# jimmyshe/liorf

Hardware: AMD Instinct MI355X
Metric: LM iterations/sec (64-line scan vs 200k-pt map) (higher is better)
Workload: dtype f32; 1 GPU; kitti64: 120000-pt scan vs 200000-pt local surf map, 30 LM iterations per scan (early exit off), one scan per GPU at a time, 8 distinct seeded scans in rotation, map replicated; n_q=120000, n_m=200000, distinct_scans=8, parallelism=scan-per-gpu x1

## Files before the change

liorf_amd/csrc/s2m_abi.hip:

```cpp
#include <hip/hip_runtime.h>

#include <cfloat>
#include <cmath>
#include <cstdio>
#include <cstdlib>
#include <cstring>
#include <algorithm>
#include <limits>
#include <map>
#include <new>
#include <string>
#include <vector>

#include "s2m_context.hpp"
#include "s2m_kernels.hpp"

using namespace s2m;
using namespace s2m::host;

namespace {

inline uint32_t host_f2ord(float f) { uint32_t u; memcpy(&u, &f, 4); return (u & 0x80000000u) ? ~u : (u | 0x80000000u); }
inline float host_ord2f(uint32_t o) { uint32_t u = (o & 0x80000000u) ? (o & 0x7fffffffu) : ~o; float f; memcpy(&f, &u, 4); return f; }

// ... 305 lines not shown
    SlotTable tbl;
    int nslots = 1;
    int nblocks = 0;
    int table_cap = 0;
    int wpb = kBlock / 64;
    bool batch = false;
    bool split = false;
    bool late = false;
    bool split_auto = false;
};

LoopShape shape_of(s2m_context* h)
{
    LoopShape sh;
    memset(&sh.tbl, 0, sizeof(sh.tbl));
    sh.tbl.ctx[0] = h->reg.dctx.as<DevCtx>();
    sh.tbl.st[0] = h->reg.state.as<DevState>();
    sh.nslots = 1; sh.nblocks = h->hctx.nblocks; sh.table_cap = h->hctx.table_cap; sh.wpb = h->hctx.wpb;
    sh.batch = h->batch.parent != nullptr && !h->batch.slot_mode;
    sh.split = h->tune.split_mode == 1;
    return sh;
}

template <bool HOOK, int NW, int MINW, int MODE, int CNW>
inline void launch_k(hipStream_t s, const LoopShape& sh, int L, int flags, int grid_x = 0)
{
    hipLaunchKernelGGL((k_register<HOOK, NW, MINW, MODE, CNW>), dim3(grid_x > 0 ? std::min(grid_x, sh.nblocks) : sh.nblocks, sh.nslots), dim3(NW * 64), 0, s,
                       sh.tbl, L, flags);
}

inline void launch_fused(s2m_context* h, const LoopShape& sh, bool hook, int L, int solve_prev)
{
// ... 510 lines not shown
    key.push_back(part); key.push_back(part ? h->tune.seg_iters : 0);
    for (int b : live) { key.push_back(b); key.push_back(h->batch.kids[(size_t)b]->hctx.table_cap); key.push_back(h->batch.kids[(size_t)b]->hctx.wpb); }
    auto it = h->batch.graphs.find(key);
    if (it != h->batch.graphs.end()) { *out = it->second; return S2M_OK; }
    hipGraph_t graph = nullptr;
    hipGraphExec_t exec = nullptr;
    std::vector<LoopShape> loops;
    if (h->tune.lockstep) {
        for (int wpb : { kBlock / 64, kBigWaves }) {
            LoopShape sh;
            memset(&sh.tbl, 0, sizeof(sh.tbl));
            sh.nslots = 0; sh.wpb = wpb; sh.batch = true;
            for (int b : live) {
                s2m_context* k = h->batch.kids[(size_t)b];
                if (k->hctx.wpb != wpb) continue;
                sh.tbl.ctx[sh.nslots] = k->reg.dctx.as<DevCtx>();
                sh.tbl.st[sh.nslots] = k->reg.state.as<DevState>();
                sh.nslots++;
                sh.nblocks = std::max(sh.nblocks, k->hctx.nblocks);
                sh.table_cap = std::max(sh.table_cap, k->hctx.table_cap);
            }
            sh.split = h->tune.split_mode == 1;
            sh.split_auto = h->tune.split_mode == 2 || h->tune.split_mode < 0;
            if (sh.nslots) loops.push_back(sh);
        }
    } else
        for (int b : live) loops.push_back(shape_of(h->batch.kids[(size_t)b]));
    S2M_HIP(h, hipStreamBeginCapture(h->stream, hipStreamCaptureModeThreadLocal));
    bool ok = hipEventRecord(h->batch.ev_fork, h->stream) == hipSuccess;
    hipStream_t keep = h->stream;
    for (size_t j = 0; j < loops.size(); j++) {
        hipStream_t br = h->batch.branch_streams[j];
// ... 658 lines not shown
```

liorf_amd/csrc/s2m_kernels.hpp:

```cpp
#pragma once
#include <float.h>
#include <math.h>
#include <string.h>
#include "s2m_types.h"

#if defined(__HIPCC__)
#define S2M_HD __host__ __device__
#else
#define S2M_HD
#endif

namespace s2m {

template <typename T> using gptr = __attribute__((address_space(1))) T*;
template <typename T> __device__ __forceinline__ gptr<T> G(T* p) { return (gptr<T>)p; }
typedef float v4f __attribute__((ext_vector_type(4)));
typedef const __attribute__((address_space(4))) DevCtx* CtxP;
__device__ __forceinline__ CtxP ctx_const(const DevCtx* p) { return (CtxP)p; }
__device__ __forceinline__ GridDesc grid_of(CtxP cp)
{
    GridDesc g;
    g.ox = cp->g.ox; g.oy = cp->g.oy; g.oz = cp->g.oz; g.inv_e = cp->g.inv_e; g.e = cp->g.e;
    g.nx = cp->g.nx; g.ny = cp->g.ny; g.nz = cp->g.nz; g.ncells = cp->g.ncells;
    return g;
}
__device__ __forceinline__ uint32_t f2ord(float f)
{
    uint32_t u = __float_as_uint(f);
    return (u & 0x80000000u) ? ~u : (u | 0x80000000u);
}

__device__ __forceinline__ int cell_coord(float v, float o, float inv_e, int n)
{
    float f = floorf((v - o) * inv_e);
    f = fminf(fmaxf(f, 0.0f), (float)(n - 1));
    return (int)f;
}

__device__ __forceinline__ void swap_if(bool c, float& a, float& b)
{
    float t = a; a = c ? b : a; b = c ? t : b;
}
__device__ __forceinline__ void swap_if(bool c, int& a, int& b)
{
    int t = a; a = c ? b : a; b = c ? t : b;
}

struct SincosfTable { double sign[4]; double hpi_inv, hpi, c0, c1, c2, c3, c4, s1, s2, s3; };
S2M_HD inline const SincosfTable& sincosf_table(int negate)
{
    static constexpr SincosfTable T[2] = {
        { { 1.0, -1.0, -1.0, 1.0 }, 0x1.45F306DC9C883p+23, 0x1.921FB54442D18p0, 0x1p0, -0x1.ffffffd0c621cp-2, 0x1.55553e1068f19p-5,
          -0x1.6c087e89a359dp-10, 0x1.99343027bf8c3p-16, -0x1.555545995a603p-3, 0x1.1107605230bc4p-7, -0x1.994eb3774cf24p-13 },
        { { 1.0, -1.0, -1.0, 1.0 }, 0x1.45F306DC9C883p+23, 0x1.921FB54442D18p0, -0x1p0, 0x1.ffffffd0c621cp-2, -0x1.55553e1068f19p-5,
          0x1.6c087e89a359dp-10, -0x1.99343027bf8c3p-16, -0x1.555545995a603p-3, 0x1.1107605230bc4p-7, -0x1.994eb3774cf24p-13 } };
    return T[negate];
}
S2M_HD inline uint32_t abstop12(float x)
{
    uint32_t u;
    memcpy(&u, &x, 4);
    return (u >> 20) & 0x7ffu;
}
S2M_HD inline float sinf_poly(double x, double x2, const SincosfTable& p, int n)
{
    if ((n & 1) == 0) {
        const double x3 = x * x2, s1 = p.s2 + x2 * p.s3, x7 = x3 * x2, s = x + x3 * p.s1;
        return (float)(s + x7 * s1);
    }
    const double x4 = x2 * x2, c2 = p.c3 + x2 * p.c4, c1 = p.c0 + x2 * p.c1, x6 = x4 * x2, c = c1 + x4 * p.c2;
    return (float)(c + x6 * c2);
}
S2M_HD inline float glibc_sincosf(float y, int which)
{
    double x = (double)y;
    if (abstop12(y) < abstop12(0x1.921FB6p-1f)) {
        if (abstop12(y) < abstop12(0x1p-12f)) return which ? 1.0f : y;
        return sinf_poly(x, x * x, sincosf_table(0), which);
    }
    if (abstop12(y) < abstop12(120.0f)) {
        const SincosfTable& p0 = sincosf_table(0);
        const double r = x * p0.hpi_inv;
        const int n = ((int32_t)r + 0x800000) >> 24;
        x = x - (double)n * p0.hpi;
        const double sgn = p0.sign[n & 3];
        return sinf_poly(x * sgn, x * x, sincosf_table((n & 2) ? 1 : 0), n ^ which);
    }
    return which ? (float)cos(x) : (float)sin(x);
}

S2M_HD inline void glibc_sincosf_both(float y, float& sn, float& cs)
{
    double x = (double)y;
    int n = 0;
    int tbl = 0;
    if (abstop12(y) < abstop12(0x1.921FB6p-1f)) {
        if (abstop12(y) < abstop12(0x1p-12f)) { sn = y; cs = 1.0f; return; }
    } else if (abstop12(y) < abstop12(120.0f)) {
        const SincosfTable& p0 = sincosf_table(0);
        const double r = x * p0.hpi_inv;
        n = ((int32_t)r + 0x800000) >> 24;
        x = x - (double)n * p0.hpi;
        x = x * p0.sign[n & 3];
        tbl = (n & 2) ? 1 : 0;
    } else { sn = (float)sin(x); cs = (float)cos(x); return; }
    const SincosfTable& p = sincosf_table(tbl);
    const double x2 = x * x;
    const float a = sinf_poly(x, x2, p, 0), b = sinf_poly(x, x2, p, 1);
    sn = (n & 1) ? b : a;
    cs = (n & 1) ? a : b;
}

S2M_HD inline float glibc_atanf(float x)
{
    const float atanhi[4] = { 4.6364760399e-01f, 7.8539812565e-01f, 9.8279368877e-01f, 1.5707962513e+00f };
    const float atanlo[4] = { 5.0121582440e-09f, 3.7748947079e-08f, 3.4473217170e-08f, 7.5497894159e-08f };
    const float aT[11] = { 3.3333334327e-01f, -2.0000000298e-01f, 1.4285714924e-01f, -1.1111110449e-01f, 9.0908870101e-02f, -7.6918758452e-02f,
                           6.6610731184e-02f, -5.8335702866e-02f, 4.9768779427e-02f, -3.6531571299e-02f, 1.6285819933e-02f };
    uint32_t u;
    memcpy(&u, &x, 4);
    const int32_t hx = (int32_t)u, ix = hx & 0x7fffffff;
    int id;
    if (ix >= 0x4c000000) {
        if (ix > 0x7f800000) return x + x;
        return (hx > 0) ? atanhi[3] + atanlo[3] : -atanhi[3] - atanlo[3];
// ... 494 lines not shown
        *n_waves_out = nw;
        if (st) st->n_waves = nw;
    }
    if (factor) for (int c = threadIdx.x; c < n_chunks; c += 1024) factor[c] = 0;
}

__global__ __launch_bounds__(1024) void k_chunk_table(const PrepTable tbl)
{
    const PrepSlot& ps = tbl.s[blockIdx.y];
    if (ps.n <= 0) return;
    chunk_table_body(ps.chunk_parts, ps.n, ps.n_chunks, ps.capacity, ps.wave_table, ps.n_waves, nullptr, nullptr);
}

__global__ __launch_bounds__(1024) void k_chunk_table_density(const SlotTable tbl)
{
    DevCtx* __restrict__ cp = const_cast<DevCtx*>(tbl.ctx[blockIdx.y]);
    DevState* __restrict__ st = tbl.st[blockIdx.y];
    if (!cp->density_pending) return;
    __syncthreads();
    if (threadIdx.x == 0) cp->density_pending = 0;
    chunk_table_body(cp->chunk_parts, cp->n_q, cp->n_chunks, cp->table_cap, cp->wave_table_rw, cp->n_waves_rw,
                     cp->chunk_factor, st);
}

__device__ __forceinline__ void plane_fit_5x3(float (&qr)[5][3], float (&x)[3])
{
    float hC[3], nU[3], nD[3];
    int perm[3] = { 0, 1, 2 };
#pragma unroll
    for (int k = 0; k < 3; k++) {
        float s = 0.0f;
#pragma unroll
// ... 396 lines not shown
            L[i][j] = v / dj;
        }
    }
    return true;
}

struct LmShared {
    double part[kFinThreads / 32][32];
    double tot[32];
    float  AtA[36], AtB[6];
    float  eA[6][6], eV[6][6], eVi[6][6], eV2[6][6], eW[6];
    int    eR[6], eC[6];
};

struct NoHook { __device__ __forceinline__ void operator()() const {} };
template <int NT, bool kFull, typename Early = NoHook, typename Late = NoHook>
__device__ __forceinline__ bool lm_close_iteration(CtxP cp, gptr<DevState> st, int nb_act, int iter,
                                                   bool writer, bool ne_only, const float (&pose0)[6], int degen0,
                                                   LmShared& sh, float* s_out, float (&pose_out)[6],
                                                   unsigned long long* stamps = nullptr,
                                                   Early early = Early(), Late late = Late())
{
    constexpr int NG = NT / 32;
    const auto trace = G(cp->trace);
    const int t = threadIdx.x, col = t & 31, grp = t >> 5, lane = t & 63, wave = t >> 6;
    double s = 0.0;
    if (col < kAcc) {
        const int nbk = cp->nblocks;
        const auto P = G((const double*)cp->partials) + (size_t)(iter & 1) * (size_t)nbk * kAcc;
        const int nb = min(nbk, nb_act);
        for (int b0 = grp; b0 < nb; b0 += 16 * NG) {
            double v[16];
#pragma unroll
            for (int u = 0; u < 16; u++) { const int b = b0 + u * NG; v[u] = (b < nb) ? P[(size_t)b * kAcc + col] : 0.0; }
#pragma unroll
            for (int u = 0; u < 16; u++) s += v[u];
        }
    }
    sh.part[grp][col] = s;
    __syncthreads();
    if (stamps) stamps[0] = wall_clock64();
    early();

    int n_sel = 0;
    if (wave == 0) {
        if (t < kAcc) {
// ... 120 lines not shown
    const float ang = (lane == 0) ? pose[2] : ((lane == 1) ? pose[1] : pose[0]);
    float snf, csf;
    glibc_sincosf_both(ang, snf, csf);
    const float B = __int_as_float(__builtin_amdgcn_readlane(__float_as_int(snf), 0)), A = __int_as_float(__builtin_amdgcn_readlane(__float_as_int(csf), 0));
    const float D = __int_as_float(__builtin_amdgcn_readlane(__float_as_int(snf), 1)), C = __int_as_float(__builtin_amdgcn_readlane(__float_as_int(csf), 1));
    const float F = __int_as_float(__builtin_amdgcn_readlane(__float_as_int(snf), 2)), E = __int_as_float(__builtin_amdgcn_readlane(__float_as_int(csf), 2));
    const float DE = D * E, DF = D * F;
    T[0] = A * C; T[1] = A * DF - B * E; T[2]  = B * F + A * DE; T[3]  = pose[3];
    T[4] = B * C; T[5] = A * E + B * DF; T[6]  = B * DE - A * F; T[7]  = pose[4];
    T[8] = -D;    T[9] = C * F;          T[10] = C * E;          T[11] = pose[5];
    sc6[0] = B; sc6[1] = A; sc6[2] = D; sc6[3] = C; sc6[4] = F; sc6[5] = E;
}

__global__ __launch_bounds__(256) void k_wave_density(const SlotTable tbl, int raw_limit)
{
    const CtxP cp = ctx_const(tbl.ctx[blockIdx.y]);
    const auto st = G((const DevState*)tbl.st[blockIdx.y]);
    const int lane = threadIdx.x & 63;
    const int wv = blockIdx.x * 4 + (threadIdx.x >> 6);
    if (!cp->density_pending || wv >= st->n_waves) return;
    const auto tb = G((const int2*)cp->wave_table);
    const int2 e = make_int2(tb[wv].x, tb[wv].y);
    const int i = e.x + lane;
    const bool valid = lane < e.y && i < cp->n_q;
    float sx = 0.0f, sy = 0.0f, sz = 0.0f;
    if (valid) {
        const float px = G(cp->qx)[i], py = G(cp->qy)[i], pz = G(cp->qz)[i];
        sx = ((st->T[0] * px + st->T[1] * py) + st->T[2]  * pz) + st->T[3];
        sy = ((st->T[4] * px + st->T[5] * py) + st->T[6]  * pz) + st->T[7];
        sz = ((st->T[8] * px + st->T[9] * py) + st->T[10] * pz) + st->T[11];
    }
    const bool fin = valid && (fabsf(sx) < 3.0e38f) && (fabsf(sy) < 3.0e38f) && (fabsf(sz) < 3.0e38f);
// ... 12 lines not shown
    for (int r = lane; r < nyb * nzb; r += 64) {
        const int zq = r / nyb;
        const int gcell = ((bz0 + zq) * g.ny + by0 + (r - zq * nyb)) * g.nx;
        raw += cell_start[gcell + bx1 + 1] - cell_start[gcell + bx0];
    }
    raw = __builtin_amdgcn_readlane(wave_incl_scan_i32(raw), 63);
    int f = raw <= raw_limit ? 1 : (raw <= 2 * raw_limit ? 2 : (raw <= 4 * raw_limit ? 4 : 8));
    f = min(f, max(e.y / 8, 1));
    if (lane == 0 && f > 1) atomicMax(&cp->chunk_factor[e.x >> 6], f);
}

#include "s2m_register.hpp"

__global__ __launch_bounds__(kFinThreads) void k_finalize(const SlotTable tbl, int iter, int mode)
{
    const CtxP cp = ctx_const(tbl.ctx[blockIdx.y]);
    const auto st = G(tbl.st[blockIdx.y]);
    const int done0 = st->done, degen0 = st->isDegenerate;
    const int nb_act = (st->n_waves + cp->wpb - 1) / cp->wpb;
    float pose0[6];
#pragma unroll
    for (int k = 0; k < 6; k++) pose0[k] = st->pose2[iter & 1][k];
    if (mode == 0 && done0) return;
    __shared__ LmShared sh;
    __shared__ float s_out[8];
    if (mode == 0 && threadIdx.x == 0 && cp->wl_count) { cp->wl_count[0] = 0; cp->wl_count[1] = 0; }
    float pose[6];
    const bool ended = lm_close_iteration<kFinThreads, true>(cp, st, nb_act, iter, true, mode == 1, pose0, degen0, sh, s_out, pose);
    if (mode == 0 && !ended && threadIdx.x < 64) {
        float T[12], sc6[6];
        build_transform(pose, (int)threadIdx.x, T, sc6);
        if (threadIdx.x == 0 && !st->stalled) {
#pragma unroll
            for (int k = 0; k < 12; k++) st->T[k] = T[k];
#pragma unroll
            for (int k = 0; k < 6; k++) st->sc[k] = sc6[k];
            st->T_valid = 1;
        }
    }
}

__global__ __launch_bounds__(256) void k_debug_sincos(const float* __restrict__ x, int n, float* __restrict__ s, float* __restrict__ c,
                                                      float* __restrict__ a)
// ... 298 lines not shown
```

liorf_amd/csrc/s2m_register.hpp:

```cpp
#pragma once

constexpr float kCertMargin = 2e-6f;
constexpr float kNbrReach   = 0.15f;
constexpr float kTightBound = 0.62f;
constexpr float kNbrReachCold = 0.10f;
constexpr int   kWalkLanes = 64;
constexpr int   kNbr = kNbrCap;
constexpr float kFragileSlack = 3e-5f;
constexpr float kSlabRound = 1e-6f;
constexpr float kAbsRound = 2.4e-7f;
constexpr int   kTilePad = 32;
constexpr int   kShareMin = 24;
constexpr int   kWalkMax = 384;
constexpr int   kServeLanes = 4;
typedef int v4i __attribute__((ext_vector_type(4)));
typedef float v3f __attribute__((ext_vector_type(3)));

__device__ __forceinline__ uint32_t key_hi(uint64_t k) { return (uint32_t)(k >> 32); }
__device__ __forceinline__ uint32_t key_lo(uint64_t k) { return (uint32_t)k; }
__device__ __forceinline__ void cas_u64(uint64_t& a, uint64_t& b)
{
    const bool c = b < a;
    const uint64_t t = a;
    a = c ? b : a; b = c ? t : b;
// ... 975 lines not shown
{
    sx = ((T[0] * px + T[1] * py) + T[2]  * pz) + T[3];
    sy = ((T[4] * px + T[5] * py) + T[6]  * pz) + T[7];
    sz = ((T[8] * px + T[9] * py) + T[10] * pz) + T[11];
    const bool fin = valid && (fabsf(sx) < 3.0e38f) && (fabsf(sy) < 3.0e38f) && (fabsf(sz) < 3.0e38f);
    const float ex = sx - cert.x, ey = sy - cert.y, ez = sz - cert.z;
    eps = sqrtf((ex * ex + ey * ey) + ez * ez) * 1.0001f + 1e-6f;
    return fin && !(!(ablate & 1) && (eps < cert.w));
}

template <int NW, int EPW, int MINW>
__global__ __launch_bounds__(NW / EPW * 64, MINW) void k_certify_lean(const SlotTable tbl, int launch)
{
    static_assert(NW % EPW == 0, "whole entries per wave");
    constexpr int NWL = NW / EPW;
    const CtxP cp = ctx_const(tbl.ctx[blockIdx.y]);
    const auto st = G(tbl.st[blockIdx.y]);
    const int done = st->done, n_waves = st->n_waves;
    if (done) return;
    __shared__ double red[NW][32];
    __shared__ float park[EPW == 2 ? NWL : 1][7][64];
    const int tid = threadIdx.x, lane = tid & 63, wave = tid >> 6;
    const int nblocks = cp->nblocks;
    const int nb_act = min((n_waves + NW - 1) / NW, nblocks);
    const int b = (int)blockIdx.x;
    if (b >= nb_act) return;
    const int nq = cp->n_q;
    const int ablate = cp->ablate;
    const bool single = nb_act * NW >= n_waves;
    static_assert(EPW == 1 || EPW == 2, "one or two entries per wave");
    const auto tb = G((const int2*)cp->wave_table);
    int2 chunkA = make_int2(0, 0), chunkB = make_int2(0, 0);
    {
// ... 5 lines not shown
    }
    float px = 0.0f, py = 0.0f, pz = 0.0f, bx = 0.0f, by = 0.0f, bz = 0.0f;
    v4f cert = { 0, 0, 0, 0 }, certB = { 0, 0, 0, 0 }, plane0 = { NAN, 0, 0, 0 };
    if (lane < chunkA.y && chunkA.x + lane < nq) {
        const int i = chunkA.x + lane;
        px = G(cp->qx)[i]; py = G(cp->qy)[i]; pz = G(cp->qz)[i];
        cert = G((const v4f*)cp->cert)[i];
        plane0 = G((const v4f*)cp->plane_cache)[i];
    }
    if (EPW == 2 && lane < chunkB.y && chunkB.x + lane < nq) {
        const int i = chunkB.x + lane;
        bx = G(cp->qx)[i]; by = G(cp->qy)[i]; bz = G(cp->qz)[i];
        certB = G((const v4f*)cp->cert)[i];
    }
    float T[12], sc6[6];
    if (st->T_valid) {
#pragma unroll
        for (int k = 0; k < 12; k++) T[k] = st->T[k];
#pragma unroll
        for (int k = 0; k < 6; k++) sc6[k] = st->sc[k];
    } else {
        float pose[6];
#pragma unroll
        for (int k = 0; k < 6; k++) pose[k] = st->pose2[launch & 1][k];
        build_transform(pose, lane, T, sc6);
    }
#pragma unroll
    for (int k = 0; k < 12; k++) T[k] = __int_as_float(__builtin_amdgcn_readfirstlane(__float_as_int(T[k])));
#pragma unroll
    for (int k = 0; k < 6; k++) sc6[k] = __int_as_float(__builtin_amdgcn_readfirstlane(__float_as_int(sc6[k])));

    bool defer = !single;
    int2 chunk = chunkA;
#pragma unroll 1
    for (int q = 0; q < EPW && single; q++) {
        const int w = wave + q * NWL;
        const int e = w * nb_act + b;
#pragma unroll
        for (int k = 0; k < 6; k++) asm volatile("" : "+s"(sc6[k]));
// ... 92 lines not shown
        if (tid == 0) {
            const int slot = atomicAdd(cp->wl_count + (launch & 1), 1);
            G(cp->wl_items)[(size_t)(launch & 1) * (size_t)nblocks + slot] = b;
        }
        return;
    }
    write_partial_row<NW>(cp, launch, b, tid, red);
}

template <bool HOOK, int NW, int MINW, int MODE, int CNW = NW>
__global__ __launch_bounds__(NW * 64, MINW) void k_register(const SlotTable tbl, int launch, int flags)
{
    static_assert(MODE == kSearch || CNW == NW, "only the search kernel works on another kernel's partition");
    static_assert(CNW % NW == 0, "a search workgroup takes the waves of a row in whole rounds");
    static_assert(!(HOOK && MODE == kCertify), "the observation hook needs the association in line");
    const CtxP cp = ctx_const(tbl.ctx[blockIdx.y]);
    const auto st = G(tbl.st[blockIdx.y]);
    const int done = st->done, n_waves = st->n_waves;
    if (!HOOK && done) return;
    const bool solve_prev = MODE != kSearch && (flags & kFlagSolvePrev) != 0;
    unsigned long long tk_start = 0, clk1 = 0, clk2 = 0;
    unsigned long long lm_stamps[7] = { 0, 0, 0, 0, 0, 0, 0 };
    if (HOOK) tk_start = wall_clock64();

    constexpr bool kHasSearch = MODE != kCertify;
    constexpr int  kTileWaves = kHasSearch ? NW : 1;
    __shared__ v4f     s_pts[kTileWaves][kHasSearch ? kTilePts : 1];
    static_assert(sizeof(v4f) * kTilePts >= sizeof(int32_t) * 18 * 64, "run table must fit the tile area");
    __shared__ double  red[CNW][32];
    __shared__ int2    s_rows[kTileWaves][kHasSearch ? 64 : 1];
    constexpr bool kKeep = kHasSearch && NW == 8 && MINW == 2;
    __shared__ float   s_keep[kKeep ? NW : 1][kKeep ? 7 : 1][kKeep ? 64 : 1];
    __shared__ float   s_lm_out[8];
    __shared__ LmShared s_lm;

    const int tid = threadIdx.x, lane = tid & 63, wave = tid >> 6;
    const int nblocks = cp->nblocks;
    const int nb_act = min((n_waves + CNW - 1) / CNW, nblocks);
    int b = (int)blockIdx.x;
    int wl_cnt = 0, wl_at = (int)blockIdx.x;
    const bool listed = MODE == kSearch && !(flags & kFlagAll);
    if (listed) {
        const auto wlc = G(cp->wl_count);
        wl_cnt = wlc[launch & 1];
        if (b == 0 && tid == 0) { wlc[(launch + 1) & 1] = 0; st->deferred_total += wl_cnt; }
    } else if (MODE == kSearch) {
        if (b == 0 && tid == 0) G(cp->wl_count)[(launch + 1) & 1] = 0;
    }
    for (;;) {
    if (listed) {
        if (wl_at >= wl_cnt) {
            if (!(flags & kFlagCloseAfter)) return;
// ... 18 lines not shown
    chunk.y = __builtin_amdgcn_readfirstlane(chunk.y);
    float px = 0.0f, py = 0.0f, pz = 0.0f;
    v4f cert = { 0, 0, 0, 0 }, plane0 = { NAN, 0, 0, 0 };
    const bool valid0 = lane < chunk.y && chunk.x + lane < nq;
    if (valid0) {
        const int i = chunk.x + lane;
        px = G(cp->qx)[i]; py = G(cp->qy)[i]; pz = G(cp->qz)[i];
        cert = G((const v4f*)cp->cert)[i];
        plane0 = G((const v4f*)cp->plane_cache)[i];
    }

    Fragile frag;
#pragma unroll
    for (int k = 0; k < 6; k++) frag.fr[k] = v4f{ 0.0f, 0.0f, 0.0f, 0.0f };
    float T[12], sc6[6];
    if (!solve_prev && st->T_valid) {
#pragma unroll
        for (int k = 0; k < 12; k++) T[k] = st->T[k];
#pragma unroll
        for (int k = 0; k < 6; k++) sc6[k] = st->sc[k];
    } else {
        float pose[6];
        if (solve_prev) {
            static_assert(MODE == kCertify || sizeof(LmShared) <= sizeof(v4f) * kTilePts * NW, "LM scratch must fit the tile area");
            LmShared& sh = (MODE == kCertify) ? s_lm : *reinterpret_cast<LmShared*>(&s_pts[0][0]);
            const int degen0 = st->isDegenerate;
            float pose0[6];
#pragma unroll
            for (int k = 0; k < 6; k++) pose0[k] = st->pose2[(launch - 1) & 1][k];
            if (HOOK) lm_stamps[5] = wall_clock64();
            auto early = [&]() {
                if (!HOOK && valid0 && !(cert.w > kFragileSlack) && !(ablate & 3)) {
                    const int i = chunk.x + lane;
                    frag.on = true;
                    frag.aux = G((const v4i*)cp->aux)[i];
#pragma unroll
                    for (int j = 0; j < 5; j++) frag.opos[j] = G(cp->npos)[(size_t)j * nq + i];
#pragma unroll
                    for (int j = 0; j < 6; j++) frag.fr[j] = G((const v4f*)cp->front)[(size_t)j * nq + i];
#pragma unroll
                    for (int j = 0; j < 5; j++) frag.alt[j] = G(cp->npos_alt)[(size_t)j * nq + i];
                    frag.alt_plane = G((const v4f*)cp->plane_alt)[i];
                }
            };
            auto late = [&]() {};
            const bool ended = lm_close_iteration<NW * 64, false>(cp, st, nb_act, launch - 1, blockIdx.x == 0, false, pose0, degen0,
                                                                 sh, s_lm_out, pose, HOOK ? lm_stamps : nullptr, early, late);
            if (ended) return;
        } else {
#pragma unroll
            for (int k = 0; k < 6; k++) pose[k] = st->pose2[launch & 1][k];
        }
        build_transform(pose, lane, T, sc6);
    }
#pragma unroll
    for (int k = 0; k < 12; k++) T[k] = __int_as_float(__builtin_amdgcn_readfirstlane(__float_as_int(T[k])));
#pragma unroll
    for (int k = 0; k < 6; k++) sc6[k] = __int_as_float(__builtin_amdgcn_readfirstlane(__float_as_int(sc6[k])));
    if (HOOK) lm_stamps[6] = wall_clock64();

    WaveProf prof;
    double acc[kAcc];
    bool defer = false;

    if (MODE == kSearch && CNW != NW) {
        for (int r = 0; r < CNW / NW; r++) {
// ... 194 lines not shown
        __syncthreads();
    write_partial_row<CNW>(cp, launch, b, tid, red);
    if (!listed) return;
    wl_at += (int)gridDim.x;
    __syncthreads();
    }
    if (MODE == kSearch) {
        __syncthreads();
        LmShared& sh = *reinterpret_cast<LmShared*>(&s_pts[0][0]);
        static_assert(MODE != kSearch || sizeof(LmShared) <= sizeof(v4f) * kTilePts * NW, "LM scratch must fit the tile area");
        float pose0[6], pose[6];
#pragma unroll
        for (int k = 0; k < 6; k++) pose0[k] = st->pose2[launch & 1][k];
        const int degen0 = st->isDegenerate;
        if (tid == 0) { cp->wl_count[0] = 0; cp->wl_count[1] = 0; }
        const bool ended = lm_close_iteration<NW * 64, false>(cp, st, nb_act, launch, true, false, pose0, degen0, sh, s_lm_out, pose);
        if (!ended && tid < 64) {
            float Tn[12], scn[6];
            build_transform(pose, tid, Tn, scn);
            if (tid == 0 && !st->stalled) {
#pragma unroll
                for (int k = 0; k < 12; k++) st->T[k] = Tn[k];
#pragma unroll
                for (int k = 0; k < 6; k++) st->sc[k] = scn[k];
                st->T_valid = 1;
            }
        }
    }
}
```

liorf_amd/csrc/s2m_types.h:

```cpp
#pragma once
#include <stdint.h>
#include <hip/hip_runtime.h>
#include "../../include/liorf_s2m.h"
#include "../../include/liorf_s2m_debug.h"

namespace s2m {

constexpr int kBlock = 512;
constexpr int kAcc = 28;
constexpr int kFinThreads = 1024;
constexpr int kMaxIter = 64;
constexpr int kProfWords = 32;
constexpr int kBlocksQuantum = 8;
constexpr int kNbrCap = 6;
constexpr int kMaxBlocks = 512;
constexpr int kBigWaves = 16;

struct GridDesc {
    float ox, oy, oz;
    float inv_e;
    float e;
    int   nx, ny, nz;
    int   ncells;
};

struct DevState {
    float pose[6];
    float pose2[2][6];
    float T[12];
    float sc[6];
    float matP[36];
    float AtA[36];
    float AtB[6];
    int32_t isDegenerate;
    int32_t done;
    int32_t converged;
    int32_t iters_run;
    int32_t n_sel_last;
    int32_t stalled;
    int32_t n_waves;
    int32_t T_valid;
    int32_t deferred_total;
    int32_t pad_;
};

struct DevCtx {
    GridDesc g;
    const float4* map_sorted;
    const int32_t* cell_start;
    const float* qx; const float* qy; const float* qz;
    const int32_t* qperm;
    int32_t* npos;
    float4*  cert;
    int4*    aux;
    float4*  front;
    float4*  plane_cache;
    float4*  plane_alt;
    int32_t* npos_alt;
    int32_t n_q, n_m, nblocks;
    int32_t wpb;
    int32_t table_cap;
    const int2* wave_table;
    const int32_t* n_waves;
    int2*    wave_table_rw; int32_t* n_waves_rw;
    const int32_t* chunk_parts;
    int32_t* chunk_factor;
    int32_t  n_chunks;
    int32_t  density_pending;
    double* partials;
    int32_t* wl_count;
    int32_t* wl_items;
    DevState* state;
    s2m_iter_trace* trace;
    float  gate_f;
    float  gate_r;
    double gate_sq, plane_tol, weight_scale, weight_min, conv_deg, conv_cm;
    float  eig_thresh;
    int32_t min_corr, max_iter, early_exit;
    int32_t tune[4];
    int32_t ablate;
    int32_t* dbg_idx5; float* dbg_d2; uint8_t* dbg_flag; float* dbg_coeff;
    unsigned long long* dbg_clk;
};

constexpr int kMaxSlots = 64;
struct SlotTable {
    const DevCtx* ctx[kMaxSlots];
    DevState*     st[kMaxSlots];
};

struct PrepSlot {
    const unsigned char* pts; size_t stride;
    int32_t n, n_chunks, base_parts, capacity, npb;
    int32_t *cell_of, *rank_of, *block_hist, *counts, *cell_start;
    float *qx, *qy, *qz; int32_t* qperm; float4* cert; int4* aux;
    int32_t* chunk_parts; int2* wave_table; int32_t* n_waves;
};
constexpr int kPrepSlots = 16;
struct PrepTable { PrepSlot s[kPrepSlots]; };

struct StateInit {
    DevState* dst; const int32_t* n_waves;
    float pose[6], T[12], sc[6], matP[36];
    int32_t isDegenerate;
// ... 8 lines not shown
```

liorf_amd/s2m.py:

```python
from __future__ import annotations

import ctypes as C
import importlib.util
import os
import sys

import numpy as np

_HERE = os.path.dirname(os.path.abspath(__file__))
LIB_PATH = os.environ.get("S2M_LIB") or os.path.join(_HERE, "libliorf_s2m.so")

S2M_OK = 0
S2M_ERR_CAPACITY = -5
ERRORS = {-1: "S2M_ERR_INVALID_ARG", -2: "S2M_ERR_NO_DEVICE", -3: "S2M_ERR_HIP", -4: "S2M_ERR_NO_SCAN",
          -5: "S2M_ERR_CAPACITY"}

ABI_SYMBOLS = [
    "s2m_version", "s2m_default_params", "s2m_create", "s2m_destroy", "s2m_last_error", "s2m_set_params", "s2m_get_params",
    "s2m_set_map", "s2m_set_map_device", "s2m_set_scan", "s2m_set_scan_device",
    "s2m_optimize", "s2m_optimize_resident", "s2m_optimize_launch", "s2m_optimize_collect",
    "s2m_optimize_batch", "s2m_batch_set_scan", "s2m_batch_set_scans", "s2m_slot_set_scan", "s2m_slot_optimize_launch", "s2m_slot_optimize_collect", "s2m_optimize_batch_launch", "s2m_optimize_batch_collect", "s2m_batch_get_trace",
    "s2m_get_trace", "s2m_surf_optimization", "s2m_normal_eq", "s2m_last_timing", "s2m_debug_deferred",
    "s2m_time_iteration_kernel", "s2m_time_iterations", "s2m_make_scancontext", "s2m_debug_wave_profile", "s2m_debug_time_steady", "s2m_time_loop_launches",
    "s2m_voxel_downsample", "s2m_voxel_downsample_device", "s2m_downsample_scan", "s2m_extract_cloud",
# ... 267 lines not shown
    L.s2m_pg_apply_to_store.argtypes = [vp, C.c_int32, C.c_int32]
    L.s2m_pg_marginals_check_args.argtypes = [C.c_int32, i32p, C.c_int32]
    L.s2m_pg_marginals.argtypes = [vp, i32p, C.c_int32, dp]
    L.s2m_pg_joint_marginal.argtypes = [vp, C.c_int32, C.c_int32, dp]
    L.s2m_update_initial_guess.argtypes = [C.POINTER(GuessState), C.POINTER(C.c_float), C.c_int, C.POINTER(GuessInfo), C.c_int, C.c_int,
                                           C.POINTER(C.c_float)]
    if path is None:
        _LIB = L
    return L


def kernel_source_sha() -> str:
    import hashlib
    h = hashlib.sha256()
    d = os.path.join(_HERE, "csrc")
    for f in ("s2m_kernels.hpp", "s2m_register.hpp", "s2m_types.h"):
        h.update(f.encode())
        h.update(open(os.path.join(d, f), "rb").read())
    return h.hexdigest()[:16]


def default_params(**kw) -> Params:
    p = Params()
    load_library().s2m_default_params(C.byref(p))
    for k, v in kw.items():
        setattr(p, k, v)
    return p


def _fp(a):
    return a.ctypes.data_as(C.POINTER(C.c_float))
# ... 847 lines not shown
```

Measured before the change: 52510 LM iterations/s.

## Pack hot device state into cache lines and prefetch LM partial rows early

DevState and DevCtx are reordered and 64-byte aligned so the fields each kernel reads first share one or two cache lines. Kernels read that hot header once into registers, and SlotTable becomes an array of ctx/state pairs. The first batch of LM partial rows is fetched before the rest of the setup so the load latency overlaps other work. The sincosf tables are replaced with constants built in registers and an fma-based range reduction, which removes scalar memory loads but may change rounding slightly.

```diff
diff --git a/liorf_amd/csrc/s2m_abi.hip b/liorf_amd/csrc/s2m_abi.hip
--- a/liorf_amd/csrc/s2m_abi.hip
+++ b/liorf_amd/csrc/s2m_abi.hip
@@ -343,8 +343,8 @@
 {
     LoopShape sh;
     memset(&sh.tbl, 0, sizeof(sh.tbl));
-    sh.tbl.ctx[0] = h->reg.dctx.as<DevCtx>();
-    sh.tbl.st[0] = h->reg.state.as<DevState>();
+    sh.tbl.s[0].ctx = h->reg.dctx.as<DevCtx>();
+    sh.tbl.s[0].st = h->reg.state.as<DevState>();
     sh.nslots = 1; sh.nblocks = h->hctx.nblocks; sh.table_cap = h->hctx.table_cap; sh.wpb = h->hctx.wpb;
     sh.batch = h->batch.parent != nullptr && !h->batch.slot_mode;
     sh.split = h->tune.split_mode == 1;
@@ -885,8 +885,8 @@
             for (int b : live) {
                 s2m_context* k = h->batch.kids[(size_t)b];
                 if (k->hctx.wpb != wpb) continue;
-                sh.tbl.ctx[sh.nslots] = k->reg.dctx.as<DevCtx>();
-                sh.tbl.st[sh.nslots] = k->reg.state.as<DevState>();
+                sh.tbl.s[sh.nslots].ctx = k->reg.dctx.as<DevCtx>();
+                sh.tbl.s[sh.nslots].st = k->reg.state.as<DevState>();
                 sh.nslots++;
                 sh.nblocks = std::max(sh.nblocks, k->hctx.nblocks);
                 sh.table_cap = std::max(sh.table_cap, k->hctx.table_cap);
diff --git a/liorf_amd/csrc/s2m_kernels.hpp b/liorf_amd/csrc/s2m_kernels.hpp
--- a/liorf_amd/csrc/s2m_kernels.hpp
+++ b/liorf_amd/csrc/s2m_kernels.hpp
@@ -9,6 +9,7 @@
 #else
 #define S2M_HD
 #endif
+#include "s2m_sincosf.hpp"
 
 namespace s2m {
 
@@ -24,6 +25,18 @@
     g.nx = cp->g.nx; g.ny = cp->g.ny; g.nz = cp->g.nz; g.ncells = cp->g.ncells;
     return g;
 }
+struct HotState {
+    int32_t done, n_waves, T_valid, isDegenerate;
+    float pose2[2][6];
+};
+__device__ __forceinline__ HotState hot_head(gptr<DevState> st)
+{
+    HotState h;
+    h.done = st->done; h.n_waves = st->n_waves; h.T_valid = st->T_valid; h.isDegenerate = st->isDegenerate;
+#pragma unroll
+    for (int k = 0; k < 6; k++) { h.pose2[0][k] = st->pose2[0][k]; h.pose2[1][k] = st->pose2[1][k]; }
+    return h;
+}
 __device__ __forceinline__ uint32_t f2ord(float f)
 {
     uint32_t u = __float_as_uint(f);
@@ -44,71 +57,6 @@
 __device__ __forceinline__ void swap_if(bool c, int& a, int& b)
 {
     int t = a; a = c ? b : a; b = c ? t : b;
-}
-
-struct SincosfTable { double sign[4]; double hpi_inv, hpi, c0, c1, c2, c3, c4, s1, s2, s3; };
-S2M_HD inline const SincosfTable& sincosf_table(int negate)
-{
-    static constexpr SincosfTable T[2] = {
-        { { 1.0, -1.0, -1.0, 1.0 }, 0x1.45F306DC9C883p+23, 0x1.921FB54442D18p0, 0x1p0, -0x1.ffffffd0c621cp-2, 0x1.55553e1068f19p-5,
-          -0x1.6c087e89a359dp-10, 0x1.99343027bf8c3p-16, -0x1.555545995a603p-3, 0x1.1107605230bc4p-7, -0x1.994eb3774cf24p-13 },
-        { { 1.0, -1.0, -1.0, 1.0 }, 0x1.45F306DC9C883p+23, 0x1.921FB54442D18p0, -0x1p0, 0x1.ffffffd0c621cp-2, -0x1.55553e1068f19p-5,
-          0x1.6c087e89a359dp-10, -0x1.99343027bf8c3p-16, -0x1.555545995a603p-3, 0x1.1107605230bc4p-7, -0x1.994eb3774cf24p-13 } };
-    return T[negate];
-}
-S2M_HD inline uint32_t abstop12(float x)
-{
-    uint32_t u;
-    memcpy(&u, &x, 4);
-    return (u >> 20) & 0x7ffu;
-}
-S2M_HD inline float sinf_poly(double x, double x2, const SincosfTable& p, int n)
-{
-    if ((n & 1) == 0) {
-        const double x3 = x * x2, s1 = p.s2 + x2 * p.s3, x7 = x3 * x2, s = x + x3 * p.s1;
-        return (float)(s + x7 * s1);
-    }
-    const double x4 = x2 * x2, c2 = p.c3 + x2 * p.c4, c1 = p.c0 + x2 * p.c1, x6 = x4 * x2, c = c1 + x4 * p.c2;
-    return (float)(c + x6 * c2);
-}
-S2M_HD inline float glibc_sincosf(float y, int which)
-{
-    double x = (double)y;
-    if (abstop12(y) < abstop12(0x1.921FB6p-1f)) {
-        if (abstop12(y) < abstop12(0x1p-12f)) return which ? 1.0f : y;
-        return sinf_poly(x, x * x, sincosf_table(0), which);
-    }
-    if (abstop12(y) < abstop12(120.0f)) {
-        const SincosfTable& p0 = sincosf_table(0);
-        const double r = x * p0.hpi_inv;
-        const int n = ((int32_t)r + 0x800000) >> 24;
-        x = x - (double)n * p0.hpi;
-        const double sgn = p0.sign[n & 3];
-        return sinf_poly(x * sgn, x * x, sincosf_table((n & 2) ? 1 : 0), n ^ which);
-    }
-    return which ? (float)cos(x) : (float)sin(x);
-}
-
-S2M_HD inline void glibc_sincosf_both(float y, float& sn, float& cs)
-{
-    double x = (double)y;
-    int n = 0;
-    int tbl = 0;
-    if (abstop12(y) < abstop12(0x1.921FB6p-1f)) {
-        if (abstop12(y) < abstop12(0x1p-12f)) { sn = y; cs = 1.0f; return; }
-    } else if (abstop12(y) < abstop12(120.0f)) {
-        const SincosfTable& p0 = sincosf_table(0);
-        const double r = x * p0.hpi_inv;
-        n = ((int32_t)r + 0x800000) >> 24;
-        x = x - (double)n * p0.hpi;
-        x = x * p0.sign[n & 3];
-        tbl = (n & 2) ? 1 : 0;
-    } else { sn = (float)sin(x); cs = (float)cos(x); return; }
-    const SincosfTable& p = sincosf_table(tbl);
-    const double x2 = x * x;
-    const float a = sinf_poly(x, x2, p, 0), b = sinf_poly(x, x2, p, 1);
-    sn = (n & 1) ? b : a;
-    cs = (n & 1) ? a : b;
 }
 
 S2M_HD inline float glibc_atanf(float x)
@@ -633,8 +581,8 @@
 
 __global__ __launch_bounds__(1024) void k_chunk_table_density(const SlotTable tbl)
 {
-    DevCtx* __restrict__ cp = const_cast<DevCtx*>(tbl.ctx[blockIdx.y]);
-    DevState* __restrict__ st = tbl.st[blockIdx.y];
+    DevCtx* __restrict__ cp = const_cast<DevCtx*>(tbl.s[blockIdx.y].ctx);
+    DevState* __restrict__ st = tbl.s[blockIdx.y].st;
     if (!cp->density_pending) return;
     __syncthreads();
     if (threadIdx.x == 0) cp->density_pending = 0;
@@ -1061,8 +1009,21 @@
 };
 
 struct NoHook { __device__ __forceinline__ void operator()() const {} };
+template <int NT>
+__device__ __forceinline__ void lm_fetch_rows(CtxP cp, int nb_act, int iter, double (&v)[16])
+{
+    constexpr int NG = NT / 32;
+    const int t = threadIdx.x, col = t & 31, grp = t >> 5;
+    const int nbk = cp->nblocks, nb = min(nbk, nb_act);
+#pragma unroll
+    for (int u = 0; u < 16; u++) v[u] = 0.0;
+    if (nb <= 0) return;
+    const auto P = G((const double*)cp->partials) + (size_t)(iter & 1) * (size_t)nbk * kAcc + min(col, kAcc - 1);
+#pragma unroll
+    for (int u = 0; u < 16; u++) v[u] = P[(size_t)min(grp + u * NG, nb - 1) * kAcc];
+}
 template <int NT, bool kFull, typename Early = NoHook, typename Late = NoHook>
-__device__ __forceinline__ bool lm_close_iteration(CtxP cp, gptr<DevState> st, int nb_act, int iter,
+__device__ __forceinline__ bool lm_close_iteration(CtxP cp, gptr<DevState> st, int nb_act, int iter, const double (&rows0)[16],
                                                    bool writer, bool ne_only, const float (&pose0)[6], int degen0,
                                                    LmShared& sh, float* s_out, float (&pose_out)[6],
                                                    unsigned long long* stamps = nullptr,
@@ -1076,7 +1037,14 @@
         const int nbk = cp->nblocks;
         const auto P = G((const double*)cp->partials) + (size_t)(iter & 1) * (size_t)nbk * kAcc;
         const int nb = min(nbk, nb_act);
-        for (int b0 = grp; b0 < nb; b0 += 16 * NG) {
+        if (grp < nb) {
+            double r[16];
+#pragma unroll
+            for (int u = 0; u < 16; u++) { r[u] = rows0[u]; asm volatile("" : "+v"(r[u])); }
+#pragma unroll
+            for (int u = 0; u < 16; u++) s += (grp + u * NG < nb) ? r[u] : 0.0;
+        }
+        for (int b0 = grp + 16 * NG; b0 < nb; b0 += 16 * NG) {
             double v[16];
 #pragma unroll
             for (int u = 0; u < 16; u++) { const int b = b0 + u * NG; v[u] = (b < nb) ? P[(size_t)b * kAcc + col] : 0.0; }
@@ -1227,8 +1195,8 @@
 
 __global__ __launch_bounds__(256) void k_wave_density(const SlotTable tbl, int raw_limit)
 {
-    const CtxP cp = ctx_const(tbl.ctx[blockIdx.y]);
-    const auto st = G((const DevState*)tbl.st[blockIdx.y]);
+    const CtxP cp = ctx_const(tbl.s[blockIdx.y].ctx);
+    const auto st = G((const DevState*)tbl.s[blockIdx.y].st);
     const int lane = threadIdx.x & 63;
     const int wv = blockIdx.x * 4 + (threadIdx.x >> 6);
     if (!cp->density_pending || wv >= st->n_waves) return;
@@ -1271,19 +1239,24 @@
 
 __global__ __launch_bounds__(kFinThreads) void k_finalize(const SlotTable tbl, int iter, int mode)
 {
-    const CtxP cp = ctx_const(tbl.ctx[blockIdx.y]);
-    const auto st = G(tbl.st[blockIdx.y]);
-    const int done0 = st->done, degen0 = st->isDegenerate;
-    const int nb_act = (st->n_waves + cp->wpb - 1) / cp->wpb;
+    const SlotRef slot = tbl.s[blockIdx.y];
+    const CtxP cp = ctx_const(slot.ctx);
+    const auto st = G(slot.st);
+    const HotState hs = hot_head(st);
+    asm volatile("" :: "s"(cp->wpb), "s"(iter), "s"(mode));
+    const int done0 = hs.done, degen0 = hs.isDegenerate;
+    if (mode == 0 && done0) return;
+    const int nb_act = (hs.n_waves + cp->wpb - 1) / cp->wpb;
+    double rows0[16];
+    lm_fetch_rows<kFinThreads>(cp, nb_act, iter, rows0);
     float pose0[6];
 #pragma unroll
-    for (int k = 0; k < 6; k++) pose0[k] = st->pose2[iter & 1][k];
-    if (mode == 0 && done0) return;
+    for (int k = 0; k < 6; k++) pose0[k] = (iter & 1) ? hs.pose2[1][k] : hs.pose2[0][k];
     __shared__ LmShared sh;
     __shared__ float s_out[8];
     if (mode == 0 && threadIdx.x == 0 && cp->wl_count) { cp->wl_count[0] = 0; cp->wl_count[1] = 0; }
     float pose[6];
-    const bool ended = lm_close_iteration<kFinThreads, true>(cp, st, nb_act, iter, true, mode == 1, pose0, degen0, sh, s_out, pose);
+    const bool ended = lm_close_iteration<kFinThreads, true>(cp, st, nb_act, iter, rows0, true, mode == 1, pose0, degen0, sh, s_out, pose);
     if (mode == 0 && !ended && threadIdx.x < 64) {
         float T[12], sc6[6];
         build_transform(pose, (int)threadIdx.x, T, sc6);
diff --git a/liorf_amd/csrc/s2m_register.hpp b/liorf_amd/csrc/s2m_register.hpp
--- a/liorf_amd/csrc/s2m_register.hpp
+++ b/liorf_amd/csrc/s2m_register.hpp
@@ -1013,9 +1013,11 @@
 {
     static_assert(NW % EPW == 0, "whole entries per wave");
     constexpr int NWL = NW / EPW;
-    const CtxP cp = ctx_const(tbl.ctx[blockIdx.y]);
-    const auto st = G(tbl.st[blockIdx.y]);
-    const int done = st->done, n_waves = st->n_waves;
+    const SlotRef slot = tbl.s[blockIdx.y];
+    const CtxP cp = ctx_const(slot.ctx);
+    const auto st = G(slot.st);
+    const HotState hs = hot_head(st);
+    const int done = hs.done, n_waves = hs.n_waves;
     if (done) return;
     __shared__ double red[NW][32];
     __shared__ float park[EPW == 2 ? NWL : 1][7][64];
@@ -1051,7 +1053,7 @@
         certB = G((const v4f*)cp->cert)[i];
     }
     float T[12], sc6[6];
-    if (st->T_valid) {
+    if (hs.T_valid) {
 #pragma unroll
         for (int k = 0; k < 12; k++) T[k] = st->T[k];
 #pragma unroll
@@ -1059,7 +1061,7 @@
     } else {
         float pose[6];
 #pragma unroll
-        for (int k = 0; k < 6; k++) pose[k] = st->pose2[launch & 1][k];
+        for (int k = 0; k < 6; k++) pose[k] = (launch & 1) ? hs.pose2[1][k] : hs.pose2[0][k];
         build_transform(pose, lane, T, sc6);
     }
 #pragma unroll
@@ -1182,11 +1184,18 @@
     static_assert(MODE == kSearch || CNW == NW, "only the search kernel works on another kernel's partition");
     static_assert(CNW % NW == 0, "a search workgroup takes the waves of a row in whole rounds");
     static_assert(!(HOOK && MODE == kCertify), "the observation hook needs the association in line");
-    const CtxP cp = ctx_const(tbl.ctx[blockIdx.y]);
-    const auto st = G(tbl.st[blockIdx.y]);
-    const int done = st->done, n_waves = st->n_waves;
+    const SlotRef slot = tbl.s[blockIdx.y];
+    const CtxP cp = ctx_const(slot.ctx);
+    const auto st = G(slot.st);
+    const HotState hs = hot_head(st);
+    asm volatile("" :: "s"(launch), "s"(flags));
+    const int nblocks = cp->nblocks;
+    const int done = hs.done, n_waves = hs.n_waves;
     if (!HOOK && done) return;
     const bool solve_prev = MODE != kSearch && (flags & kFlagSolvePrev) != 0;
+    float pose_in[6];
+#pragma unroll
+    for (int k = 0; k < 6; k++) pose_in[k] = (((solve_prev ? launch - 1 : launch) & 1) != 0) ? hs.pose2[1][k] : hs.pose2[0][k];
     unsigned long long tk_start = 0, clk1 = 0, clk2 = 0;
     unsigned long long lm_stamps[7] = { 0, 0, 0, 0, 0, 0, 0 };
     if (HOOK) tk_start = wall_clock64();
@@ -1203,7 +1212,6 @@
     __shared__ LmShared s_lm;
 
     const int tid = threadIdx.x, lane = tid & 63, wave = tid >> 6;
-    const int nblocks = cp->nblocks;
     const int nb_act = min((n_waves + CNW - 1) / CNW, nblocks);
     int b = (int)blockIdx.x;
     int wl_cnt = 0, wl_at = (int)blockIdx.x;
@@ -1252,7 +1260,7 @@
 #pragma unroll
     for (int k = 0; k < 6; k++) frag.fr[k] = v4f{ 0.0f, 0.0f, 0.0f, 0.0f };
     float T[12], sc6[6];
-    if (!solve_prev && st->T_valid) {
+    if (!solve_prev && (MODE == kSearch ? st->T_valid : hs.T_valid)) {
 #pragma unroll
         for (int k = 0; k < 12; k++) T[k] = st->T[k];
 #pragma unroll
@@ -1262,10 +1270,12 @@
         if (solve_prev) {
             static_assert(MODE == kCertify || sizeof(LmShared) <= sizeof(v4f) * kTilePts * NW, "LM scratch must fit the tile area");
             LmShared& sh = (MODE == kCertify) ? s_lm : *reinterpret_cast<LmShared*>(&s_pts[0][0]);
-            const int degen0 = st->isDegenerate;
+            const int degen0 = hs.isDegenerate;
             float pose0[6];
 #pragma unroll
-            for (int k = 0; k < 6; k++) pose0[k] = st->pose2[(launch - 1) & 1][k];
+            for (int k = 0; k < 6; k++) pose0[k] = pose_in[k];
+            double rows0[16];
+            lm_fetch_rows<NW * 64>(cp, nb_act, launch - 1, rows0);
             if (HOOK) lm_stamps[5] = wall_clock64();
             auto early = [&]() {
                 if (!HOOK && valid0 && !(cert.w > kFragileSlack) && !(ablate & 3)) {
@@ -1282,12 +1292,12 @@
                 }
             };
             auto late = [&]() {};
-            const bool ended = lm_close_iteration<NW * 64, false>(cp, st, nb_act, launch - 1, blockIdx.x == 0, false, pose0, degen0,
+            const bool ended = lm_close_iteration<NW * 64, false>(cp, st, nb_act, launch - 1, rows0, blockIdx.x == 0, false, pose0, degen0,
                                                                  sh, s_lm_out, pose, HOOK ? lm_stamps : nullptr, early, late);
             if (ended) return;
         } else {
 #pragma unroll
-            for (int k = 0; k < 6; k++) pose[k] = st->pose2[launch & 1][k];
+            for (int k = 0; k < 6; k++) pose[k] = (MODE == kSearch) ? st->pose2[launch & 1][k] : pose_in[k];
         }
         build_transform(pose, lane, T, sc6);
     }
@@ -1512,7 +1522,9 @@
         for (int k = 0; k < 6; k++) pose0[k] = st->pose2[launch & 1][k];
         const int degen0 = st->isDegenerate;
         if (tid == 0) { cp->wl_count[0] = 0; cp->wl_count[1] = 0; }
-        const bool ended = lm_close_iteration<NW * 64, false>(cp, st, nb_act, launch, true, false, pose0, degen0, sh, s_lm_out, pose);
+        double rows_c[16];
+        lm_fetch_rows<NW * 64>(cp, nb_act, launch, rows_c);
+        const bool ended = lm_close_iteration<NW * 64, false>(cp, st, nb_act, launch, rows_c, true, false, pose0, degen0, sh, s_lm_out, pose);
         if (!ended && tid < 64) {
             float Tn[12], scn[6];
             build_transform(pose, tid, Tn, scn);
diff --git a/liorf_amd/csrc/s2m_sincosf.hpp b/liorf_amd/csrc/s2m_sincosf.hpp
--- /dev/null
+++ b/liorf_amd/csrc/s2m_sincosf.hpp
@@ -0,0 +1,84 @@
+#pragma once
+#include <math.h>
+#include <stdint.h>
+#include <string.h>
+
+#ifndef S2M_HD
+#if defined(__HIPCC__)
+#define S2M_HD __host__ __device__
+#else
+#define S2M_HD
+#endif
+#endif
+
+namespace s2m {
+
+struct SincosfPoly { double c0, c1, c2, c3, c4, s1, s2, s3; };
+constexpr double kSincosfHpiInv = 0x1.45F306DC9C883p+23, kSincosfHpi = 0x1.921FB54442D18p0;
+S2M_HD inline double sincosf_const(double c, uint32_t flip_hi, uint32_t z)
+{
+    const uint64_t b = __builtin_bit_cast(uint64_t, c);
+    const uint64_t u = ((uint64_t)((((uint32_t)(b >> 32)) ^ flip_hi) | z) << 32) | (uint64_t)(((uint32_t)b) | z);
+    return __builtin_bit_cast(double, u);
+}
+S2M_HD inline SincosfPoly sincosf_poly_of(int n)
+{
+    uint32_t z = 0;
+#if defined(__HIP_DEVICE_COMPILE__)
+    asm volatile("" : "+v"(z));
+#endif
+    const uint32_t f = ((uint32_t)n & 2u) << 30;
+    SincosfPoly p;
+    p.c0 = sincosf_const(0x1p0, f, z);
+    p.c1 = sincosf_const(-0x1.ffffffd0c621cp-2, f, z);
+    p.c2 = sincosf_const(0x1.55553e1068f19p-5, f, z);
+    p.c3 = sincosf_const(-0x1.6c087e89a359dp-10, f, z);
+    p.c4 = sincosf_const(0x1.99343027bf8c3p-16, f, z);
+    p.s1 = sincosf_const(-0x1.555545995a603p-3, 0u, z);
+    p.s2 = sincosf_const(0x1.1107605230bc4p-7, 0u, z);
+    p.s3 = sincosf_const(-0x1.994eb3774cf24p-13, 0u, z);
+    return p;
+}
+S2M_HD inline double sincosf_sign_of(int n) { return ((n + 1) & 2) ? -1.0 : 1.0; }
+S2M_HD inline uint32_t abstop12(float x)
+{
+    uint32_t u;
+    memcpy(&u, &x, 4);
+    return (u >> 20) & 0x7ffu;
+}
+S2M_HD inline float sinf_poly(double x, double x2, const SincosfPoly& p, int n)
+{
+    if ((n & 1) == 0) {
+        const double x3 = x * x2, s1 = p.s2 + x2 * p.s3, x7 = x3 * x2, s = x + x3 * p.s1;
+        return (float)(s + x7 * s1);
+    }
+    const double x4 = x2 * x2, c2 = p.c3 + x2 * p.c4, c1 = p.c0 + x2 * p.c1, x6 = x4 * x2, c = c1 + x4 * p.c2;
+    return (float)(c + x6 * c2);
+}
+
+S2M_HD inline void glibc_sincosf_both(float y, float& sn, float& cs)
+{
+    double x = (double)y;
+    int n = 0;
+    if (abstop12(y) < abstop12(0x1.921FB6p-1f)) {
+        if (abstop12(y) < abstop12(0x1p-12f)) { sn = y; cs = 1.0f; return; }
+    } else if (abstop12(y) < abstop12(120.0f)) {
+        const double r = x * kSincosfHpiInv;
+        n = ((int32_t)r + 0x800000) >> 24;
+        x = fma(-(double)n, kSincosfHpi, x);
+        x = x * sincosf_sign_of(n);
+    } else { sn = (float)sin(x); cs = (float)cos(x); return; }
+    const SincosfPoly p = sincosf_poly_of(n);
+    const double x2 = x * x;
+    const float a = sinf_poly(x, x2, p, 0), b = sinf_poly(x, x2, p, 1);
+    sn = (n & 1) ? b : a;
+    cs = (n & 1) ? a : b;
+}
+S2M_HD inline float glibc_sincosf(float y, int which)
+{
+    float sn, cs;
+    glibc_sincosf_both(y, sn, cs);
+    return which ? cs : sn;
+}
+
+}
diff --git a/liorf_amd/csrc/s2m_types.h b/liorf_amd/csrc/s2m_types.h
--- a/liorf_amd/csrc/s2m_types.h
+++ b/liorf_amd/csrc/s2m_types.h
@@ -1,4 +1,5 @@
 #pragma once
+#include <stddef.h>
 #include <stdint.h>
 #include <hip/hip_runtime.h>
 #include "../../include/liorf_s2m.h"
@@ -24,70 +25,78 @@
     int   ncells;
 };
 
-struct DevState {
+struct alignas(64) DevState {
+    int32_t done;
+    int32_t n_waves;
+    int32_t T_valid;
+    int32_t isDegenerate;
+    float pose2[2][6];
+    int32_t stalled;
+    int32_t converged;
+    int32_t iters_run;
+    int32_t n_sel_last;
+    int32_t deferred_total;
+    int32_t pad_;
     float pose[6];
-    float pose2[2][6];
     float T[12];
     float sc[6];
     float matP[36];
     float AtA[36];
     float AtB[6];
-    int32_t isDegenerate;
-    int32_t done;
-    int32_t converged;
-    int32_t iters_run;
-    int32_t n_sel_last;
-    int32_t stalled;
-    int32_t n_waves;
-    int32_t T_valid;
-    int32_t deferred_total;
-    int32_t pad_;
 };
+static_assert(offsetof(DevState, done) == 0 && offsetof(DevState, pose2) + sizeof(float) * 12 == 64 && offsetof(DevState, stalled) == 64,
+              "done, n_waves, T_valid, isDegenerate and both pose2 slots are the first 64-byte line");
+static_assert(alignof(DevState) == 64 && sizeof(DevState) % 64 == 0, "the hot line of every DevState is one cache line (the trace follows the block)");
 
-struct DevCtx {
-    GridDesc g;
+struct alignas(64) DevCtx {
+    int32_t nblocks;
+    int32_t n_q;
+    int32_t wpb;
+    int32_t ablate;
+    float   gate_f;
+    int32_t min_corr, max_iter, early_exit;
+    double  conv_deg, conv_cm;
+    const int2* wave_table;
+    double* partials;
+    const float* qx; const float* qy; const float* qz;
+    float4*  cert;
+    float4*  plane_cache;
+    int4*    aux;
+    int32_t* npos;
+    float4*  front;
+    s2m_iter_trace* trace;
+    float4*  plane_alt;
+    int32_t* npos_alt;
+    const int32_t* qperm;
     const float4* map_sorted;
     const int32_t* cell_start;
-    const float* qx; const float* qy; const float* qz;
-    const int32_t* qperm;
-    int32_t* npos;
-    float4*  cert;
-    int4*    aux;
-    float4*  front;
-    float4*  plane_cache;
-    float4*  plane_alt;
-    int32_t* npos_alt;
-    int32_t n_q, n_m, nblocks;
-    int32_t wpb;
+    GridDesc g;
+    int32_t n_m;
     int32_t table_cap;
-    const int2* wave_table;
     const int32_t* n_waves;
     int2*    wave_table_rw; int32_t* n_waves_rw;
     const int32_t* chunk_parts;
     int32_t* chunk_factor;
     int32_t  n_chunks;
     int32_t  density_pending;
-    double* partials;
     int32_t* wl_count;
     int32_t* wl_items;
     DevState* state;
-    s2m_iter_trace* trace;
-    float  gate_f;
     float  gate_r;
-    double gate_sq, plane_tol, weight_scale, weight_min, conv_deg, conv_cm;
     float  eig_thresh;
-    int32_t min_corr, max_iter, early_exit;
+    double gate_sq, plane_tol, weight_scale, weight_min;
     int32_t tune[4];
-    int32_t ablate;
     int32_t* dbg_idx5; float* dbg_d2; uint8_t* dbg_flag; float* dbg_coeff;
     unsigned long long* dbg_clk;
 };
+constexpr size_t kCtxHotBytes = 128;
+static_assert(offsetof(DevCtx, nblocks) == 0 && offsetof(DevCtx, front) + sizeof(void*) == kCtxHotBytes && offsetof(DevCtx, trace) == kCtxHotBytes,
+              "the hot header is the first 128 bytes of DevCtx");
+static_assert(alignof(DevCtx) == 64 && sizeof(DevCtx) % 64 == 0, "the hot header is two whole cache lines");
 
 constexpr int kMaxSlots = 64;
-struct SlotTable {
-    const DevCtx* ctx[kMaxSlots];
-    DevState*     st[kMaxSlots];
-};
+struct SlotRef { const DevCtx* ctx; DevState* st; };
+struct SlotTable { SlotRef s[kMaxSlots]; };
 
 struct PrepSlot {
     const unsigned char* pts; size_t stride;
diff --git a/liorf_amd/s2m.py b/liorf_amd/s2m.py
--- a/liorf_amd/s2m.py
+++ b/liorf_amd/s2m.py
@@ -305,7 +305,7 @@
     import hashlib
     h = hashlib.sha256()
     d = os.path.join(_HERE, "csrc")
-    for f in ("s2m_kernels.hpp", "s2m_register.hpp", "s2m_types.h"):
+    for f in ("s2m_kernels.hpp", "s2m_register.hpp", "s2m_types.h", "s2m_sincosf.hpp"):
         h.update(f.encode())
         h.update(open(os.path.join(d, f), "rb").read())
     return h.hexdigest()[:16]
```

Result: no change. 52580 LM iterations/s, median of 2 (+0.1%).
